# qiaozhijian/LPD-Net-Pytorch

Measured on AMD Instinct MI355X. Metric: global descriptors/sec (4096-pt clouds), higher is better.
Workload: dtype f32; 1 GPU; BASELINE configs[1]: LPD-Net (featnet=lpdnet, emb_dims=1024, no T-Nets) eval forward, N=4096, k=20, eval_batch_size=32 clouds/step/GPU; num_points=4096, batches_in_flight=2, parallelism=shard-by-cloud x1 (one process per GPU, no data-path collective)

## Files before the change

lpd-net-pytorch_amd/csrc/lpd_knn.hip:

```cpp
#include "lpd_common.h"
#include <math.h>
#include <type_traits>

namespace {

constexpr int KNN_WAVES = 4;
constexpr int KNN_THREADS = KNN_WAVES * 64;
constexpr int KNN_QPB = KNN_WAVES * 32;

template <int CP>
struct KnnCfg {
    static constexpr int CHUNK = (CP <= 32) ? 128 : (CP <= 64 ? 64 : 32);
    static constexpr int ROWS = 2 * CP;
    static constexpr int FLOATS = ROWS * CHUNK;
    static constexpr int PER_THREAD = FLOATS / KNN_THREADS;
};

__global__ void knn_sumsq_kernel(const float* __restrict__ x, float* __restrict__ xx, int C, int N)
{
    int n = blockIdx.x * blockDim.x + threadIdx.x;
    int b = blockIdx.y;
    if (n >= N) return;
    const float* p = x + (size_t)b * C * N + n;
    float total = 0.0f;
// ... 337 lines not shown
        knn_prep_bf16x8 e;
#pragma unroll
        for (int i = 0; i < 8; ++i) e[i] = (__bf16)0.0f;
        if (j == 0) {
            const float w = -0.5f * total;
            const __bf16 hi = (__bf16)w;
            e[0] = hi;
            e[1] = (__bf16)(w - (float)hi);
        }
        __bf16* f4 = xb + ((((size_t)b * nt + (pt >> 5)) * 5 + 4) * 64 + (pt & 31) + 32 * j) * 8;
        *reinterpret_cast<knn_prep_bf16x8*>(f4) = e;
    }
}

template <int CP>
__device__ __forceinline__ void knn3_ld_ops(const float* __restrict__ xpb, int N, int j, int h, float (&a)[CP])
{
    const float* row = xpb + ((size_t)min(j, N - 1) * 2 + h) * CP;
    if constexpr (CP % 4 == 0) {
#pragma unroll
        for (int g = 0; g < CP / 4; ++g) {
            const float4 v = *reinterpret_cast<const float4*>(row + 4 * g);
            a[4 * g + 0] = v.x; a[4 * g + 1] = v.y; a[4 * g + 2] = v.z; a[4 * g + 3] = v.w;
        }
    } else {
        const float2 v = *reinterpret_cast<const float2*>(row);
        a[0] = v.x; a[1] = v.y;
    }
}

__device__ __forceinline__ void knn3_ld_xx(const float* __restrict__ xxb, int N, int j0, int h, bool vec_ok, float4 (&x4)[4])
{
    if (vec_ok && j0 + 32 <= N) {
#pragma unroll
        for (int g = 0; g < 4; ++g) x4[g] = *reinterpret_cast<const float4*>(xxb + j0 + 8 * g + 4 * h);
        return;
    }
    const float nanv = __builtin_nanf("");
#pragma unroll
    for (int g = 0; g < 4; ++g) {
        const int r0 = j0 + 8 * g + 4 * h;
        x4[g].x = r0 + 0 < N ? xxb[r0 + 0] : nanv;
        x4[g].y = r0 + 1 < N ? xxb[r0 + 1] : nanv;
        x4[g].z = r0 + 2 < N ? xxb[r0 + 2] : nanv;
        x4[g].w = r0 + 3 < N ? xxb[r0 + 3] : nanv;
    }
}

template <int CP, bool ALWAYS = false>
__device__ __forceinline__ void knn3_tile(float (&a)[CP], float4 (&x4)[4], const float (&qreg)[CP], float xq,
                                          const float* __restrict__ xpb, const float* __restrict__ xxb, int N, int j_next,
                                          bool have_next, int col, int h, bool vec_ok, float (&pd)[16])
{
    if constexpr (ALWAYS) have_next = true;
    f32x16 acc = {0, 0, 0, 0, 0, 0, 0, 0, 0, 0, 0, 0, 0, 0, 0, 0};
    const float* row = xpb + ((size_t)min(j_next + col, N - 1) * 2 + h) * CP;
    if constexpr (CP % 4 == 0) {
#pragma unroll
        for (int g = 0; g < CP / 4; ++g) {
#pragma unroll
            for (int e = 0; e < 4; ++e)
                acc = __builtin_amdgcn_mfma_f32_32x32x2f32(a[4 * g + e], qreg[4 * g + e], acc, 0, 0, 0);
            if (have_next) {
                const float4 v = *reinterpret_cast<const float4*>(row + 4 * g);
                a[4 * g + 0] = v.x; a[4 * g + 1] = v.y; a[4 * g + 2] = v.z; a[4 * g + 3] = v.w;
            }
        }
    } else {
#pragma unroll
        for (int s = 0; s < CP; ++s) acc = __builtin_amdgcn_mfma_f32_32x32x2f32(a[s], qreg[s], acc, 0, 0, 0);
        if (have_next) {
            const float2 v = *reinterpret_cast<const float2*>(row);
            a[0] = v.x; a[1] = v.y;
        }
    }
#pragma unroll
    for (int r = 0; r < 16; ++r) {
        const float4 xv = x4[r >> 2];
        const float xxj = (r & 3) == 0 ? xv.x : (r & 3) == 1 ? xv.y : (r & 3) == 2 ? xv.z : xv.w;
        pd[r] = __fsub_rn(__fmaf_rn(2.0f, acc[r], -xxj), xq);
    }
    if constexpr (ALWAYS) {
#pragma unroll
        for (int g = 0; g < 4; ++g) x4[g] = *reinterpret_cast<const float4*>(xxb + j_next + 8 * g + 4 * h);
    } else if (have_next) knn3_ld_xx(xxb, N, j_next, h, vec_ok, x4);
}

template <int CP, int KMAX>
__global__ __launch_bounds__(KNN3_THREADS, ((KMAX > 32 || (KMAX == 32 && CP == 32)) ? 1 : 2))
void knn3_kernel(const float* __restrict__ xp, const float* __restrict__ xx, int32_t* __restrict__ idx, int N, int k,
                 int blocks_per_cloud, int dbg)
{
    extern __shared__ __attribute__((aligned(16))) float smem[];
    const int tid = threadIdx.x;
    const int lane = tid & 63;
    const int wave = tid >> 6;
    const int h = lane >> 5;
    const int col = lane & 31;
    const int vb = lpd_xcd_remap(blockIdx.x, gridDim.x);
    const int b = vb / blocks_per_cloud;
    const int qb = vb - b * blocks_per_cloud;
    const int q0 = qb * (KNN3_WAVES * 32) + wave * 32;
    const int q = q0 + col;
    const bool q_ok = q < N;
    const float* xpb = xp + (size_t)b * N * (2 * CP);
    const float* xxb = xx + (size_t)b * N;
    const bool vec_ok = (N & 3) == 0;
    float2* myq = reinterpret_cast<float2*>(smem + (size_t)wave * knn3_wave_floats<KMAX>()) + lane;

    float qreg[CP];
    knn3_ld_ops<CP>(xpb, N, q, h, qreg);
    const float xq = xxb[min(q, N - 1)];

    float lv[KMAX];
    int li[KMAX];
    auto reset_lists = [&]() {
#pragma unroll
        for (int s = 0; s < KMAX; ++s) {
            lv[s] = -INFINITY;
            li[s] = 0x7fffffff;
        }
    };
    reset_lists();

    const int ntiles = (N + 31) / 32;
    float a[CP];
    float4 x4[4];
    float pd[16];

    {
        const int t_own = q0 / 32;
        int t_lo = t_own - 1, t_hi = t_own + 2;
        while ((t_hi - t_lo) * 16 < KMAX) { --t_lo; ++t_hi; }
        if (t_lo < 0) { t_hi -= t_lo; t_lo = 0; }
        if (t_hi > ntiles) { t_lo -= t_hi - ntiles; t_hi = ntiles; }
        if (t_lo < 0) t_lo = 0;
        knn3_ld_ops<CP>(xpb, N, t_lo * 32 + col, h, a);
        knn3_ld_xx(xxb, N, t_lo * 32, h, vec_ok, x4);
        for (int t = t_lo; t < t_hi; ++t) {
            knn3_tile<CP>(a, x4, qreg, xq, xpb, xxb, N, (t + 1) * 32, t + 1 < t_hi, col, h, vec_ok, pd);
#pragma unroll
            for (int r = 0; r < 16; ++r) knn_insert_values<KMAX>(lv, pd[r] > lv[KMAX - 1] ? pd[r] : -INFINITY);
        }
    }
    float t0 = k <= KMAX ? lv[KMAX - 1] : -INFINITY;
    {
        const float other = __shfl_xor(t0, 32, 64);
        t0 = fmaxf(t0, other);
        if (!(t0 > -INFINITY)) t0 = -INFINITY;
    }
    reset_lists();

    int cnt = 0;
    int stat_adm = 0, stat_it = 0, stat_pass = 0;
    auto drain = [&]() {
        stat_adm += cnt;
        int nmax = cnt;
#pragma unroll
        for (int m = 32; m >= 1; m >>= 1) nmax = max(nmax, __shfl_xor(nmax, m, 64));
        nmax = __builtin_amdgcn_readfirstlane(nmax);
        for (int e = 0; e < nmax; ++e) {
            ++stat_it;
            const float2 ent = myq[(e < cnt ? e : 0) * 64];
            const float pv = (e < cnt && ent.x > lv[KMAX - 1]) ? ent.x : -INFINITY;
            knn_insert_inplace<KMAX>(lv, li, pv, __float_as_int(ent.y));
        }
        cnt = 0;
    };
    knn3_ld_ops<CP>(xpb, N, col, h, a);
    knn3_ld_xx(xxb, N, 0, h, vec_ok, x4);
    for (int t = 0; t < ntiles; ++t) {
        knn3_tile<CP>(a, x4, qreg, xq, xpb, xxb, N, (t + 1) * 32, (t + 1 < ntiles), col, h, vec_ok, pd);
        const float thr = fmaxf(t0, lv[KMAX - 1]);
        const bool list_full = lv[KMAX - 1] > -INFINITY;
        float mx = fmaxf(fmaxf(fmaxf(pd[0], pd[1]), fmaxf(pd[2], pd[3])), fmaxf(fmaxf(pd[4], pd[5]), fmaxf(pd[6], pd[7])));
        mx = fmaxf(mx, fmaxf(fmaxf(fmaxf(pd[8], pd[9]), fmaxf(pd[10], pd[11])), fmaxf(fmaxf(pd[12], pd[13]), fmaxf(pd[14], pd[15]))));
        if (!__any(list_full ? (mx > thr) : (mx >= thr))) continue;
        ++stat_pass;
#pragma unroll
        for (int r = 0; r < 16; ++r) {
            const bool admit = list_full ? (pd[r] > thr) : (pd[r] >= thr);
            if (admit) {
                const int row = (r & 3) + 8 * (r >> 2) + 4 * h;
                myq[cnt * 64] = make_float2(pd[r], __int_as_float(t * 32 + row));
                ++cnt;
            }
        }
        if (__any(cnt > KNN3_QCAP - 16)) drain();
    }
    drain();

    float* mv = smem + (size_t)wave * knn3_wave_floats<KMAX>();
    int* mi = reinterpret_cast<int*>(mv + 64 * KMAX);
#pragma unroll
    for (int s = 0; s < KMAX; ++s) {
        mv[lane * KMAX + s] = lv[s];
        mi[lane * KMAX + s] = li[s];
    }
    __syncthreads();
    if ((dbg & 64) && q_ok) {
        if (h == 0) { int32_t* o = idx + ((size_t)b * N + q) * k; o[0] = stat_adm; o[1] = stat_it; o[2] = stat_pass; o[3] = __float_as_int(t0); }
        else { int32_t* o = idx + ((size_t)b * N + q) * k; o[4] = stat_adm; }
    } else
    if (h == 0 && q_ok) {
        const float* av = mv + lane * KMAX;
        const int* ai = mi + lane * KMAX;
        const float* bv = mv + (lane + 32) * KMAX;
        const int* bi = mi + (lane + 32) * KMAX;
        int pa = 0, pb = 0;
        int32_t* out = idx + ((size_t)b * N + q) * k;
        for (int s = 0; s < k; ++s) {
            bool take_a;
            if (pa >= KMAX) take_a = false;
            else if (pb >= KMAX) take_a = true;
            else {
                const float va = av[pa], vb2 = bv[pb];
                take_a = (va > vb2) || (va == vb2 && ai[pa] < bi[pb]);
            }
            if (take_a) out[s] = ai[pa++];
            else out[s] = bi[pb++];
        }
    }
}

constexpr bool KNN7_DEFAULT = true;
constexpr int KNN7_QCAP = 24;
constexpr int KNN7_MAXT = 128;
constexpr int KNN7_WAVE_LDS = KNN7_MAXT * 32 * 2 + KNN7_QCAP * 64 * 8;
constexpr int KNN7_QCAP_XYZ = 20;
constexpr int KNN7_QCAP_BIG = 48;
constexpr int KNN7_WAVE_LDS_XYZ = KNN7_QCAP_XYZ * 64 * 8;
constexpr bool KNN7_ONFLY64 = false;
template <int CP, int KMAX, bool ONFLY> struct Knn7Cfg {
    static constexpr int QCAP = KMAX > 20 ? (CP == 2 ? 32 : KNN7_QCAP_BIG) : ((CP == 2) ? KNN7_QCAP_XYZ : KNN7_QCAP);
    static constexpr int QBYTES = QCAP * 64 * 8;
    static constexpr int TBYTES = ONFLY ? 0 : KNN7_MAXT * 32 * 2;
    static constexpr int MERGE = KMAX > 20 ? 0 : 64 * KMAX * 8;
    static constexpr int WAVE = (TBYTES + QBYTES) > MERGE ? (TBYTES + QBYTES) : MERGE;
    static constexpr int QOFF = TBYTES;
    static constexpr int WAVES_PER_SIMD = KMAX > 20 ? (CP == 2 ? 2 : 1) : (CP == 2 ? 4 : 2);
};

__device__ __forceinline__ bool knn_before(float av, int ai, float bv, int bi) { return av > bv || (av == bv && ai < bi); }

__device__ __forceinline__ void knn_merge_halves_bitonic(float (&v)[64], int (&id)[64])
{
#pragma unroll
    for (int s = 0; s < 32; ++s) {
        const int r = 63 - s;
        const float pv_r = __shfl_xor(v[r], 32, 64), pv_s = __shfl_xor(v[s], 32, 64);
        const int pi_r = __shfl_xor(id[r], 32, 64), pi_s = __shfl_xor(id[s], 32, 64);
        const bool ks = knn_before(v[s], id[s], pv_r, pi_r);
        const bool kr = knn_before(v[r], id[r], pv_s, pi_s);
        v[s] = ks ? v[s] : pv_r; id[s] = ks ? id[s] : pi_r;
        v[r] = kr ? v[r] : pv_s; id[r] = kr ? id[r] : pi_s;
    }
#pragma unroll
    for (int d = 32; d >= 1; d >>= 1)
#pragma unroll
        for (int s = 0; s < 64; ++s)
            if ((s & d) == 0) {
                const bool sw = knn_before(v[s + d], id[s + d], v[s], id[s]);
                const float tv = v[s]; const int ti = id[s];
                v[s] = sw ? v[s + d] : tv; id[s] = sw ? id[s + d] : ti;
                v[s + d] = sw ? tv : v[s + d]; id[s + d] = sw ? ti : id[s + d];
            }
}

constexpr int KNN7_XB = 80;
constexpr int KNN7_PRE_MAXT = 512;
typedef __bf16 knn_bf16x8 __attribute__((ext_vector_type(8)));

__global__ __launch_bounds__(256) void knn7_bf16_kernel(const float* __restrict__ xp, const float* __restrict__ xx, __bf16* __restrict__ xb,
                                                        int N, int nt)
{
    const int t = blockIdx.x * blockDim.x + threadIdx.x;
    if (t >= nt * 64) return;
    const int b = blockIdx.y;
    const int T = t >> 6, lane = t & 63, h = lane >> 5;
    const int pt = min(T * 32 + (lane & 31), N - 1);
    const float* src = xp + (((size_t)b * N + pt) * 2 + h) * 32;
    __bf16* dst = xb + (((size_t)b * nt + T) * 5 * 64 + lane) * 8;
#pragma unroll
    for (int g = 0; g < 4; ++g) {
        const float4 a = *reinterpret_cast<const float4*>(src + 8 * g), c = *reinterpret_cast<const float4*>(src + 8 * g + 4);
        knn_bf16x8 v;
        v[0] = (__bf16)a.x; v[1] = (__bf16)a.y; v[2] = (__bf16)a.z; v[3] = (__bf16)a.w;
        v[4] = (__bf16)c.x; v[5] = (__bf16)c.y; v[6] = (__bf16)c.z; v[7] = (__bf16)c.w;
        *reinterpret_cast<knn_bf16x8*>(dst + (size_t)g * 512) = v;
    }
    knn_bf16x8 e;
#pragma unroll
    for (int i = 0; i < 8; ++i) e[i] = (__bf16)0.0f;
    if (h == 0) {
        const float v = -0.5f * xx[(size_t)b * N + pt];
        const __bf16 hi = (__bf16)v;
        e[0] = hi;
        e[1] = (__bf16)(v - (float)hi);
    }
    *reinterpret_cast<knn_bf16x8*>(dst + (size_t)4 * 512) = e;
}

constexpr int KNN7_BQT = 2;
__global__ __launch_bounds__(256, 2) void knn7_bound_kernel(const __bf16* __restrict__ xb, const float* __restrict__ xx,
                                                            const float* __restrict__ txmax, uint16_t* __restrict__ ubq, int N, int nt, int C,
                                                            int tchunk)
{
    constexpr int QT = KNN7_BQT;
    const int tid = threadIdx.x, lane = tid & 63, wave = tid >> 6;
    const int h = lane >> 5, col = lane & 31;
    const int b = blockIdx.y;
    const int W0 = (blockIdx.x * 4 + wave) * QT;
    const __bf16* xbb = xb + ((size_t)b * nt * 5 * 64 + lane) * 8;
    const float* txb = txmax + (size_t)b * nt;
    float smax = 0.f;
    for (int t = lane; t < nt; t += 64) smax = fmaxf(smax, txb[t]);
#pragma unroll
    for (int m = 32; m >= 1; m >>= 1) smax = fmaxf(smax, __shfl_xor(smax, m, 64));
    const float E0 = 8.0f * (float)(C + 8) * 1.1920929e-7f * smax + 1e-30f;

    knn_bf16x8 qop[QT][4], ones;
    float xq[QT], kq[QT];
#pragma unroll
    for (int e = 0; e < 8; ++e) ones[e] = (__bf16)((h == 0 && e < 2) ? 1.0f : 0.0f);
#pragma unroll
    for (int i = 0; i < QT; ++i) {
        const int Wq = min(W0 + i, nt - 1);
#pragma unroll
        for (int s = 0; s < 4; ++s) qop[i][s] = *reinterpret_cast<const knn_bf16x8*>(xbb + ((size_t)Wq * 5 + s) * 512);
        xq[i] = xx[(size_t)b * N + min(Wq * 32 + col, N - 1)];
        kq[i] = (sqrtf(xq[i]) * 1.0001f + 1e-30f) * 7.9e-3f;
    }
    float pinf = INFINITY;
    asm volatile("" : "+v"(pinf));
    auto mx2 = [&](float a_, float b_) { return __builtin_amdgcn_fmed3f(a_, b_, pinf); };
    constexpr int RING = 4;
    knn_bf16x8 cop[RING][5];
    auto load_c = [&](int T, knn_bf16x8 (&c)[5]) {
        T = T < nt ? T : nt - 1;
#pragma unroll
        for (int s = 0; s < 5; ++s) c[s] = *reinterpret_cast<const knn_bf16x8*>(xbb + ((size_t)T * 5 + s) * 512);
    };
    __shared__ float stx[KNN7_PRE_MAXT];
    for (int t = tid; t < nt; t += 256) stx[t] = txb[t];
    __syncthreads();
    if (W0 >= nt) return;
    auto one_tile = [&](int T, const knn_bf16x8 (&c)[5]) {
        const float tx = stx[T];
        const float ncT = sqrtf(tx) * 1.0001f;
        const float cT = 2.0f * (tx * 7.62939453125e-6f + E0);
#pragma unroll
        for (int i = 0; i < QT; ++i) {
            f32x16 sa = {0, 0, 0, 0, 0, 0, 0, 0, 0, 0, 0, 0, 0, 0, 0, 0};
#pragma unroll
            for (int s = 0; s < 4; ++s) sa = __builtin_amdgcn_mfma_f32_32x32x16_bf16(c[s], qop[i][s], sa, 0, 0, 0);
            sa = __builtin_amdgcn_mfma_f32_32x32x16_bf16(c[4], ones, sa, 0, 0, 0);
            float m = mx2(mx2(mx2(sa[0], sa[1]), mx2(sa[2], sa[3])), mx2(mx2(sa[4], sa[5]), mx2(sa[6], sa[7])));
            m = mx2(m, mx2(mx2(mx2(sa[8], sa[9]), mx2(sa[10], sa[11])), mx2(mx2(sa[12], sa[13]), mx2(sa[14], sa[15]))));
            m = mx2(m, __shfl_xor(m, 32, 64));
            float ub = 2.0f * m - xq[i] + (2.0f * (kq[i] * ncT) + cT);
            ub += fabsf(ub) * 9.5367431640625e-7f;
            uint32_t bits = __float_as_uint(ub);
            bits = (ub <= 0.0f) ? (bits >> 16) : 0x7f80u;
            if (h == 0 && W0 + i < nt) ubq[(((size_t)b * nt + (W0 + i)) * nt + T) * 32 + col] = (uint16_t)bits;
        }
    };
    const int tbeg = blockIdx.z * tchunk, tend = min(nt, tbeg + tchunk);
#pragma unroll
    for (int d = 0; d < RING - 1; ++d) load_c(tbeg + d, cop[d]);
    for (int T0 = tbeg; T0 < tend; T0 += RING) {
#pragma unroll
        for (int d = 0; d < RING; ++d) {
            load_c(T0 + d + RING - 1, cop[(d + RING - 1) % RING]);
            if (T0 + d < tend) one_tile(T0 + d, cop[d]);
        }
    }
}

template <int CP>
__global__ __launch_bounds__(64) void knn7_tile_stats_kernel(const float* __restrict__ xp, const float* __restrict__ xx,
                                                            float* __restrict__ cenp, float* __restrict__ cnorm,
                                                            float* __restrict__ rad, float* __restrict__ txmax, int N, int nt)
{
    constexpr int CH = 2 * CP;
    __shared__ float cen[CH];
    const int t = blockIdx.x, b = blockIdx.y, tid = threadIdx.x;
    const int cnt = min(32, N - t * 32);
    const float* base = xp + ((size_t)b * N + (size_t)t * 32) * CH;
    for (int c = tid; c < CH; c += 64) {
        float sum = 0.f;
        for (int i = 0; i < cnt; ++i) sum += base[(size_t)i * CH + c];
        const float m = sum / (float)cnt;
        cen[c] = m;
        cenp[((size_t)b * nt + t) * CH + c] = m;
    }
    __syncthreads();
    float d2 = 0.f, nx = 0.f, cn = 0.f;
    if (tid < cnt) {
        for (int c = 0; c < CH; ++c) {
            const float d = base[(size_t)tid * CH + c] - cen[c];
            d2 = fmaf(d, d, d2);
        }
        nx = xx[(size_t)b * N + t * 32 + tid];
    }
    for (int c = tid; c < CH; c += 64) cn = fmaf(cen[c], cen[c], cn);
#pragma unroll
    for (int m = 32; m >= 1; m >>= 1) {
        d2 = fmaxf(d2, __shfl_xor(d2, m, 64));
        nx = fmaxf(nx, __shfl_xor(nx, m, 64));
        cn += __shfl_xor(cn, m, 64);
    }
    const bool bad = __any(tid < cnt && !(fabsf(xx[(size_t)b * N + t * 32 + tid]) <= 3.0e38f));
    if (tid == 0) {
        rad[(size_t)b * nt + t] = sqrtf(d2) * 1.0001f + 1e-30f;
        cnorm[(size_t)b * nt + t] = cn;
        txmax[(size_t)b * nt + t] = bad ? INFINITY : nx;
    }
}

template <int CP>
__global__ __launch_bounds__(128) void knn7_predict_kernel(const float* __restrict__ cenp, const float* __restrict__ rad,
                                                           int32_t* __restrict__ pred, int nt)
{
    constexpr int CH = 2 * CP;
    __shared__ float cw[CH];
    __shared__ int part[2];
    const int W = blockIdx.x, b = blockIdx.y, tid = threadIdx.x;
    const float* cb = cenp + (size_t)b * nt * CH;
    for (int c = tid; c < CH; c += 128) cw[c] = cb[(size_t)W * CH + c];
    __syncthreads();
    const float rw = rad[(size_t)b * nt + W];
    int n = 0;
    for (int T = tid; T < nt; T += 128) {
        const float* ct = cb + (size_t)T * CH;
        float d2 = 0.f;
        if constexpr (CH % 4 == 0) {
#pragma unroll 4
            for (int c = 0; c < CH; c += 4) {
                const float4 v = *reinterpret_cast<const float4*>(ct + c);
                const float d0 = v.x - cw[c], d1 = v.y - cw[c + 1], d2_ = v.z - cw[c + 2], d3 = v.w - cw[c + 3];
                d2 = fmaf(d0, d0, fmaf(d1, d1, fmaf(d2_, d2_, fmaf(d3, d3, d2))));
            }
        } else {
            for (int c = 0; c < CH; ++c) { const float d = ct[c] - cw[c]; d2 = fmaf(d, d, d2); }
        }
        const float gap = fmaxf(sqrtf(d2) - rw - rad[(size_t)b * nt + T], 0.0f);
        n += gap <= 0.5f * rw ? 1 : 0;
    }
#pragma unroll
    for (int m = 32; m >= 1; m >>= 1) n += __shfl_xor(n, m, 64);
    if ((tid & 63) == 0) part[tid >> 6] = n;
    __syncthreads();
    if (tid == 0) pred[(size_t)b * nt + W] = part[0] + part[1];
}

constexpr int KNN7_PRED_WPB = 16;
template <int CP>
__global__ __launch_bounds__(256) void knn7_predict_lds_kernel(const float* __restrict__ cenp, const float* __restrict__ rad,
                                                               int32_t* __restrict__ pred, int nt)
{
    constexpr int CH = 2 * CP, LD = CH + 1;
    extern __shared__ float pcen[];
    float* prad = pcen + (size_t)nt * LD;
    const int b = blockIdx.y, tid = threadIdx.x;
    const float* cb = cenp + (size_t)b * nt * CH;
    for (int i = tid; i < nt * CH; i += 256) pcen[(i / CH) * LD + (i % CH)] = cb[i];
    for (int i = tid; i < nt; i += 256) prad[i] = rad[(size_t)b * nt + i];
    __syncthreads();
    const int W = blockIdx.x * KNN7_PRED_WPB + (tid >> 4), l = tid & 15;
    const int Wc = min(W, nt - 1);
    const float* cw = pcen + (size_t)Wc * LD;
    const float rw = prad[Wc];
    int n = 0;
    for (int T = l; T < nt; T += 16) {
        const float* ct = pcen + (size_t)T * LD;
        float d2 = 0.f;
#pragma unroll 16
        for (int c = 0; c < CH; ++c) { const float d = ct[c] - cw[c]; d2 = fmaf(d, d, d2); }
        const float gap = fmaxf(sqrtf(d2) - rw - prad[T], 0.0f);
        n += gap <= 0.5f * rw ? 1 : 0;
    }
#pragma unroll
    for (int m = 8; m >= 1; m >>= 1) n += __shfl_xor(n, m, 64);
    if (l == 0 && W < nt) pred[(size_t)b * nt + W] = n;
}

__global__ __launch_bounds__(1024) void knn7_order_kernel(const int32_t* __restrict__ pred, int32_t* __restrict__ order, int nitems)
{
    __shared__ unsigned sk[1024];
    const int tid = threadIdx.x, xcd = blockIdx.y;
    const int q = nitems / 8, r = nitems % 8;
    const int base = xcd < r ? xcd * (q + 1) : r * (q + 1) + (xcd - r) * q;
    const int len = q + (xcd < r ? 1 : 0);
    const int c0 = blockIdx.x * 1024;
    if (c0 >= len) return;
    const int cl = min(1024, len - c0);
    unsigned v = ~0u;
    if (tid < cl) v = ((0xffffu - (unsigned)min(pred[base + c0 + tid], 0xfffe)) << 16) | (unsigned)tid;
    for (int k = 2; k <= 1024; k <<= 1) {
        for (int j = k >> 1; j > 0; j >>= 1) {
            unsigned o;
            if (j < 64) o = __shfl_xor(v, j, 64);
            else {
                sk[tid] = v;
                __syncthreads();
                o = sk[tid ^ j];
                __syncthreads();
            }
            const bool lower = (tid & j) == 0, up = (tid & k) == 0;
            const unsigned mn = v < o ? v : o, mx = v < o ? o : v;
            v = (lower == up) ? mn : mx;
        }
    }
    if (tid < cl) order[base + c0 + tid] = base + c0 + (int)(v & 0xffffu);
}

template <int KMAX>
__device__ __forceinline__ void knn7_insert(float (&v)[KMAX], int (&id)[KMAX], float x, float y, int j)
{
    unsigned long long cc, cp;
    int ti;
    asm volatile("v_cmp_ge_f32_e64 %0, %1, %2" : "=s"(cc) : "v"(v[KMAX - 1]), "v"(y));
#pragma unroll
    for (int s = KMAX - 1; s >= 1; --s) {
        asm volatile(
            "v_cmp_ge_f32_e64 %[cp], %[vp], %[y]\n\t"
            "v_med3_f32 %[vs], %[vp], %[vs], %[x]\n\t"
            "s_nop 0\n\t"
            "v_cndmask_b32_e64 %[ti], %[ip], %[j], %[cp]\n\t"
            "v_cndmask_b32_e64 %[is], %[ti], %[is], %[cc]"
            : [vs] "+v"(v[s]), [is] "+v"(id[s]), [cp] "=&s"(cp), [ti] "=&v"(ti)
            : [vp] "v"(v[s - 1]), [ip] "v"(id[s - 1]), [x] "v"(x), [y] "v"(y), [j] "v"(j), [cc] "s"(cc));
        cc = cp;
    }
    asm volatile(
        "v_cndmask_b32_e64 %[i0], %[j], %[i0], %[cc]\n\t"
        "v_max_f32 %[v0], %[v0], %[x]"
        : [v0] "+v"(v[0]), [i0] "+v"(id[0])
        : [x] "v"(x), [j] "v"(j), [cc] "s"(cc));
}

constexpr unsigned KNN_IMG_NINF = 0x00800000u;
constexpr unsigned KNN_IMG_EMPTY = 0u;
constexpr unsigned KNN_LOW_EMPTY = 0x80000000u;

__device__ __forceinline__ unsigned knn_img(float pd)
{
    const unsigned b = __float_as_uint(pd);
    return (int)b < 0 ? 0u - b : b ^ 0x80000000u;
}
__device__ __forceinline__ float knn_img_inv(unsigned im)
{
    im = im < KNN_IMG_NINF ? KNN_IMG_NINF : im;
    return __uint_as_float((im & 0x80000000u) ? im ^ 0x80000000u : 0u - im);
}

#define KNN_SUB_(n)  "v_sub_co_u32_e64 %[t], %[m" #n "], %[xl" #n "], %[yl" #n "]\n\t"
#define KNN_SBB_(n)  "v_subb_co_u32_e64 %[t], %[m" #n "], %[xh" #n "], %[yh" #n "], %[m" #n "]\n\t"
#define KNN_SELX_(n) "v_cndmask_b32_e64 %[nl" #n "], %[xl" #n "], %[yl" #n "], %[m" #n "]\n\t" \
                     "v_cndmask_b32_e64 %[nh" #n "], %[xh" #n "], %[yh" #n "], %[m" #n "]\n\t"
#define KNN_SELY_(n) "v_cndmask_b32_e64 %[yl" #n "], %[yl" #n "], %[xl" #n "], %[m" #n "]\n\t" \
                     "v_cndmask_b32_e64 %[yh" #n "], %[yh" #n "], %[xh" #n "], %[m" #n "]\n\t"
#define KNN_SELM_(n) "v_cndmask_b32_e64 %[xl" #n "], %[xl" #n "], %[yl" #n "], %[m" #n "]\n\t" \
                     "v_cndmask_b32_e64 %[xh" #n "], %[xh" #n "], %[yh" #n "], %[m" #n "]\n\t"
#define KNN_CXOUT_(n) [nl##n] "=&v"(nl##n), [nh##n] "=&v"(nh##n), [yl##n] "+v"(yl##n), [yh##n] "+v"(yh##n), [m##n] "=&s"(m##n)
#define KNN_CXIN_(n)  [xl##n] "v"(xl##n), [xh##n] "v"(xh##n)
#define KNN_MXOUT_(n) [xl##n] "+v"(xl##n), [xh##n] "+v"(xh##n), [m##n] "=&s"(m##n)
#define KNN_MXIN_(n)  [yl##n] "v"(yl##n), [yh##n] "v"(yh##n)
#define KNN_KEYREF_(n) unsigned &xh##n, unsigned &xl##n, unsigned &yh##n, unsigned &yl##n

__device__ __forceinline__ void knn_cx3(KNN_KEYREF_(0), KNN_KEYREF_(1), KNN_KEYREF_(2))
{
    unsigned long long m0, m1, m2;
    unsigned t, nl0, nh0, nl1, nh1, nl2, nh2;
    asm(KNN_SUB_(0) KNN_SUB_(1) KNN_SUB_(2) KNN_SBB_(0) KNN_SBB_(1) KNN_SBB_(2)
        KNN_SELX_(0) KNN_SELY_(0) KNN_SELX_(1) KNN_SELY_(1) KNN_SELX_(2) KNN_SELY_(2)
        : KNN_CXOUT_(0), KNN_CXOUT_(1), KNN_CXOUT_(2), [t] "=&v"(t)
        : KNN_CXIN_(0), KNN_CXIN_(1), KNN_CXIN_(2));
    xl0 = nl0; xh0 = nh0; xl1 = nl1; xh1 = nh1; xl2 = nl2; xh2 = nh2;
}
__device__ __forceinline__ void knn_cx2(KNN_KEYREF_(0), KNN_KEYREF_(1))
{
    unsigned long long m0, m1;
    unsigned t, nl0, nh0, nl1, nh1;
    asm(KNN_SUB_(0) KNN_SUB_(1) "s_nop 0\n\t" KNN_SBB_(0) KNN_SBB_(1) "s_nop 0\n\t"
        KNN_SELX_(0) KNN_SELY_(0) KNN_SELX_(1) KNN_SELY_(1)
        : KNN_CXOUT_(0), KNN_CXOUT_(1), [t] "=&v"(t)
        : KNN_CXIN_(0), KNN_CXIN_(1));
    xl0 = nl0; xh0 = nh0; xl1 = nl1; xh1 = nh1;
}
__device__ __forceinline__ void knn_cx1(KNN_KEYREF_(0))
{
    unsigned long long m0;
    unsigned t, nl0, nh0;
    asm(KNN_SUB_(0) "s_nop 1\n\t" KNN_SBB_(0) "s_nop 1\n\t" KNN_SELX_(0) KNN_SELY_(0)
        : KNN_CXOUT_(0), [t] "=&v"(t)
        : KNN_CXIN_(0));
    xl0 = nl0; xh0 = nh0;
}
__device__ __forceinline__ void knn_mx3(KNN_KEYREF_(0), KNN_KEYREF_(1), KNN_KEYREF_(2))
{
    unsigned long long m0, m1, m2;
    unsigned t;
    asm(KNN_SUB_(0) KNN_SUB_(1) KNN_SUB_(2) KNN_SBB_(0) KNN_SBB_(1) KNN_SBB_(2) KNN_SELM_(0) KNN_SELM_(1) KNN_SELM_(2)
        : KNN_MXOUT_(0), KNN_MXOUT_(1), KNN_MXOUT_(2), [t] "=&v"(t)
        : KNN_MXIN_(0), KNN_MXIN_(1), KNN_MXIN_(2));
}
__device__ __forceinline__ void knn_mx2(KNN_KEYREF_(0), KNN_KEYREF_(1))
{
    unsigned long long m0, m1;
    unsigned t;
    asm(KNN_SUB_(0) KNN_SUB_(1) "s_nop 0\n\t" KNN_SBB_(0) KNN_SBB_(1) "s_nop 0\n\t" KNN_SELM_(0) KNN_SELM_(1)
        : KNN_MXOUT_(0), KNN_MXOUT_(1), [t] "=&v"(t)
        : KNN_MXIN_(0), KNN_MXIN_(1));
}
__device__ __forceinline__ void knn_mx1(KNN_KEYREF_(0))
{
    unsigned long long m0;
    unsigned t;
    asm(KNN_SUB_(0) "s_nop 1\n\t" KNN_SBB_(0) "s_nop 1\n\t" KNN_SELM_(0)
        : KNN_MXOUT_(0), [t] "=&v"(t)
        : KNN_MXIN_(0));
}
#define KNN_K_(a, i) a##h[i], a##l[i]
#define KNN_CX3(a, i, b, j, c, k, d, l, e, m, f, n) knn_cx3(KNN_K_(a, i), KNN_K_(b, j), KNN_K_(c, k), KNN_K_(d, l), KNN_K_(e, m), KNN_K_(f, n))
#define KNN_CX2(a, i, b, j, c, k, d, l) knn_cx2(KNN_K_(a, i), KNN_K_(b, j), KNN_K_(c, k), KNN_K_(d, l))
#define KNN_CX1(a, i, b, j) knn_cx1(KNN_K_(a, i), KNN_K_(b, j))
#define KNN_MX3(a, i, b, j, c, k, d, l, e, m, f, n) knn_mx3(KNN_K_(a, i), KNN_K_(b, j), KNN_K_(c, k), KNN_K_(d, l), KNN_K_(e, m), KNN_K_(f, n))
#define KNN_MX2(a, i, b, j, c, k, d, l) knn_mx2(KNN_K_(a, i), KNN_K_(b, j), KNN_K_(c, k), KNN_K_(d, l))
#define KNN_MX1(a, i, b, j) knn_mx1(KNN_K_(a, i), KNN_K_(b, j))
#define KNN_PLACE(...) { constexpr int pl[20] = {__VA_ARGS__}; unsigned th[20], tl[20]; \
    _Pragma("unroll") for (int s = 0; s < 20; ++s) { th[s] = kh[pl[s]]; tl[s] = kl[pl[s]]; } \
    _Pragma("unroll") for (int s = 0; s < 20; ++s) { kh[s] = th[s]; kl[s] = tl[s]; } }

template <int NB> __device__ __forceinline__ void knn_merge_batch(unsigned (&kh)[20], unsigned (&kl)[20], unsigned (&bh)[NB], unsigned (&bl)[NB]);
template <> __device__ __forceinline__ void knn_merge_batch<8>(unsigned (&kh)[20], unsigned (&kl)[20], unsigned (&bh)[8], unsigned (&bl)[8])
{
    KNN_CX3(b, 0, b, 1,  b, 2, b, 3,  b, 4, b, 5);
    KNN_CX3(b, 6, b, 7,  b, 0, b, 2,  b, 1, b, 3);
    KNN_CX3(b, 4, b, 6,  b, 5, b, 7,  b, 1, b, 2);
    KNN_CX3(b, 5, b, 6,  b, 0, b, 4,  b, 3, b, 7);
    KNN_CX2(b, 1, b, 5,  b, 2, b, 6);
    KNN_CX2(b, 2, b, 4,  b, 3, b, 5);
    KNN_CX3(b, 1, b, 2,  b, 3, b, 4,  b, 5, b, 6);
    KNN_MX3(k, 12, b, 7,  k, 13, b, 6,  k, 14, b, 5);
    KNN_MX3(k, 15, b, 4,  k, 16, b, 3,  k, 17, b, 2);
    KNN_MX2(k, 18, b, 1,  k, 19, b, 0);
    KNN_CX3(k, 0, k, 16,  k, 1, k, 17,  k, 2, k, 18);
    KNN_CX3(k, 3, k, 19,  k, 16, k, 8,  k, 17, k, 9);
    KNN_CX3(k, 18, k, 10,  k, 19, k, 11,  k, 4, k, 12);
    KNN_CX3(k, 5, k, 13,  k, 6, k, 14,  k, 7, k, 15);
    KNN_CX3(k, 16, k, 4,  k, 17, k, 5,  k, 18, k, 6);
    KNN_CX3(k, 19, k, 7,  k, 8, k, 12,  k, 9, k, 13);
    KNN_CX3(k, 10, k, 14,  k, 11, k, 15,  k, 0, k, 2);
    KNN_CX3(k, 1, k, 3,  k, 16, k, 18,  k, 17, k, 19);
    KNN_CX3(k, 4, k, 6,  k, 5, k, 7,  k, 8, k, 10);
    KNN_CX3(k, 9, k, 11,  k, 12, k, 14,  k, 13, k, 15);
    KNN_CX3(k, 0, k, 1,  k, 2, k, 3,  k, 16, k, 17);
    KNN_CX3(k, 18, k, 19,  k, 4, k, 5,  k, 6, k, 7);
    KNN_CX3(k, 8, k, 9,  k, 10, k, 11,  k, 12, k, 13);
    KNN_CX1(k, 14, k, 15);
    KNN_PLACE(0, 1, 2, 3, 16, 17, 18, 19, 4, 5, 6, 7, 8, 9, 10, 11, 12, 13, 14, 15);
}
template <> __device__ __forceinline__ void knn_merge_batch<16>(unsigned (&kh)[20], unsigned (&kl)[20], unsigned (&bh)[16], unsigned (&bl)[16])
{
    KNN_CX3(b, 0, b, 1,  b, 2, b, 3,  b, 4, b, 5);
    KNN_CX3(b, 6, b, 7,  b, 8, b, 9,  b, 10, b, 11);
    KNN_CX3(b, 12, b, 13,  b, 14, b, 15,  b, 0, b, 2);
    KNN_CX3(b, 1, b, 3,  b, 4, b, 6,  b, 5, b, 7);
    KNN_CX3(b, 8, b, 10,  b, 9, b, 11,  b, 12, b, 14);
    KNN_CX3(b, 13, b, 15,  b, 1, b, 2,  b, 5, b, 6);
    KNN_CX3(b, 9, b, 10,  b, 13, b, 14,  b, 0, b, 4);
    KNN_CX3(b, 1, b, 5,  b, 2, b, 6,  b, 3, b, 7);
    KNN_CX3(b, 8, b, 12,  b, 9, b, 13,  b, 10, b, 14);
    KNN_CX3(b, 11, b, 15,  b, 2, b, 4,  b, 3, b, 5);
    KNN_CX3(b, 10, b, 12,  b, 11, b, 13,  b, 1, b, 2);
    KNN_CX3(b, 3, b, 4,  b, 5, b, 6,  b, 9, b, 10);
    KNN_CX3(b, 11, b, 12,  b, 13, b, 14,  b, 0, b, 8);
    KNN_CX3(b, 1, b, 9,  b, 2, b, 10,  b, 3, b, 11);
// ... 847 lines not shown
```

Baseline: 19860 descriptors/s.

## Software-pipeline kNN bound kernel with double-buffered MFMA accumulators and buffer loads

Restructures the kNN tile upper-bound kernel so that each step issues the MFMAs for the next tile while finishing the max-reduction and store for the previous tile, using two alternating accumulator sets. Per-tile constants are precomputed once into shared memory as float2. Global loads and stores go through raw buffer resources. The cross-half-wave shuffle is replaced by permlane32_swap, so each half-wave handles one query tile's store. Explicit sched_group_barrier hints interleave MFMA and VALU work. The aim is to hide MFMA latency and cut address and shuffle overhead, at the cost of more registers and a hand-written tail.

```diff
diff --git a/lpd-net-pytorch_amd/csrc/lpd_knn.hip b/lpd-net-pytorch_amd/csrc/lpd_knn.hip
--- a/lpd-net-pytorch_amd/csrc/lpd_knn.hip
+++ b/lpd-net-pytorch_amd/csrc/lpd_knn.hip
@@ -663,16 +663,85 @@
 }
 
 constexpr int KNN7_BQT = 2;
+constexpr int KNN7_BRING = 4;
+
+struct Knn7BoundCtx {
+    knn_bf16x8 qop[KNN7_BQT][4], ones;
+    float xqh, kqh, pinf;
+    const float2* sct;
+    __amdgpu_buffer_rsrc_t xres, ures;
+    unsigned xoff, uoff;
+    int nt;
+};
+
+__device__ __forceinline__ float knn7_mx2(const Knn7BoundCtx& k, float a, float b) { return __builtin_amdgcn_fmed3f(a, b, k.pinf); }
+
+__device__ __forceinline__ void knn7_bound_load(const Knn7BoundCtx& k, int T, knn_bf16x8 (&c)[5])
+{
+    T = T < k.nt ? T : k.nt - 1;
+#pragma unroll
+    for (int s = 0; s < 5; ++s) c[s] = __builtin_bit_cast(knn_bf16x8, __builtin_amdgcn_raw_buffer_load_b128(k.xres, k.xoff, (unsigned)(T * 5 + s) * 1024u, 0));
+}
+
+__device__ __forceinline__ void knn7_bound_mma(const Knn7BoundCtx& k, const knn_bf16x8 (&c)[5], f32x16 (&a)[KNN7_BQT])
+{
+#pragma unroll
+    for (int i = 0; i < KNN7_BQT; ++i) {
+        f32x16 sa = {0, 0, 0, 0, 0, 0, 0, 0, 0, 0, 0, 0, 0, 0, 0, 0};
+#pragma unroll
+        for (int s = 0; s < 4; ++s) sa = __builtin_amdgcn_mfma_f32_32x32x16_bf16(c[s], k.qop[i][s], sa, 0, 0, 0);
+        a[i] = __builtin_amdgcn_mfma_f32_32x32x16_bf16(c[4], k.ones, sa, 0, 0, 0);
+    }
+}
+
+__device__ __forceinline__ float knn7_bound_max16(const Knn7BoundCtx& k, const f32x16& sa)
+{
+    float p[8];
+#pragma unroll
+    for (int j = 0; j < 8; ++j) p[j] = knn7_mx2(k, sa[2 * j], sa[2 * j + 1]);
+    const float a = fmaxf(fmaxf(p[0], p[1]), p[2]), b = fmaxf(fmaxf(p[3], p[4]), p[5]);
+    return fmaxf(fmaxf(a, b), fmaxf(p[6], p[7]));
+}
+
+__device__ __forceinline__ void knn7_bound_finish(const Knn7BoundCtx& k, int T, const f32x16 (&a)[KNN7_BQT])
+{
+    const float m0 = knn7_bound_max16(k, a[0]), m1 = knn7_bound_max16(k, a[1]);
+    const auto r = __builtin_amdgcn_permlane32_swap(__float_as_uint(m0), __float_as_uint(m1), false, false);
+    const float m = knn7_mx2(k, __uint_as_float(r[0]), __uint_as_float(r[1]));
+    const float2 ct = k.sct[T];
+    float ub = fmaf(2.0f, m, -k.xqh) + fmaf(2.0f, k.kqh * ct.x, ct.y);
+    ub += fabsf(ub) * 9.5367431640625e-7f;
+    uint32_t bits = __float_as_uint(ub);
+    bits = (ub <= 0.0f) ? (bits >> 16) : 0x7f80u;
+    __builtin_amdgcn_raw_buffer_store_b16((unsigned short)bits, k.ures, k.uoff, (unsigned)T * 64u, 0);
+}
+
+template <bool LOAD>
+__device__ __forceinline__ void knn7_bound_step(const Knn7BoundCtx& k, int T, knn_bf16x8 (&cl)[5], const knn_bf16x8 (&c)[5],
+                                                f32x16 (&an)[KNN7_BQT], const f32x16 (&ap)[KNN7_BQT])
+{
+    if constexpr (LOAD) knn7_bound_load(k, T + KNN7_BRING, cl);
+    knn7_bound_mma(k, c, an);
+    knn7_bound_finish(k, T, ap);
+    __builtin_amdgcn_sched_group_barrier(0x100, 1, 0);
+#pragma unroll
+    for (int i = 0; i < 5 * KNN7_BQT; ++i) {
+        __builtin_amdgcn_sched_group_barrier(0x8, 1, 0);
+        __builtin_amdgcn_sched_group_barrier(0x2, 5, 0);
+    }
+}
+
 __global__ __launch_bounds__(256, 2) void knn7_bound_kernel(const __bf16* __restrict__ xb, const float* __restrict__ xx,
                                                             const float* __restrict__ txmax, uint16_t* __restrict__ ubq, int N, int nt, int C,
                                                             int tchunk)
 {
-    constexpr int QT = KNN7_BQT;
-    const int tid = threadIdx.x, lane = tid & 63, wave = tid >> 6;
+    constexpr int QT = KNN7_BQT, RING = KNN7_BRING;
+    static_assert(QT == 2 && RING % 2 == 0, "two query tiles (one per half-wave at the store); accumulator sets alternate with the ring");
+    const int tid = threadIdx.x, lane = tid & 63;
+    const int wave = __builtin_amdgcn_readfirstlane(tid >> 6);
     const int h = lane >> 5, col = lane & 31;
     const int b = blockIdx.y;
     const int W0 = (blockIdx.x * 4 + wave) * QT;
-    const __bf16* xbb = xb + ((size_t)b * nt * 5 * 64 + lane) * 8;
     const float* txb = txmax + (size_t)b * nt;
     float smax = 0.f;
     for (int t = lane; t < nt; t += 64) smax = fmaxf(smax, txb[t]);
@@ -680,62 +749,55 @@
     for (int m = 32; m >= 1; m >>= 1) smax = fmaxf(smax, __shfl_xor(smax, m, 64));
     const float E0 = 8.0f * (float)(C + 8) * 1.1920929e-7f * smax + 1e-30f;
 
-    knn_bf16x8 qop[QT][4], ones;
-    float xq[QT], kq[QT];
-#pragma unroll
-    for (int e = 0; e < 8; ++e) ones[e] = (__bf16)((h == 0 && e < 2) ? 1.0f : 0.0f);
+    __shared__ float2 sct[KNN7_PRE_MAXT];
+    for (int t = tid; t < nt; t += 256) {
+        const float tx = txb[t];
+        sct[t] = make_float2(sqrtf(tx) * 1.0001f, 2.0f * (tx * 7.62939453125e-6f + E0));
+    }
+    __syncthreads();
+    if (W0 >= nt) return;
+
+    Knn7BoundCtx k;
+    k.nt = nt;
+    k.sct = sct;
+    k.xres = __builtin_amdgcn_make_buffer_rsrc(reinterpret_cast<unsigned char*>(const_cast<__bf16*>(xb)) + (size_t)b * nt * 5 * 1024, 0,
+                                               (unsigned)nt * 5 * 1024, 0x00020000);
+    k.xoff = lane * 16;
+#pragma unroll
+    for (int e = 0; e < 8; ++e) k.ones[e] = (__bf16)((h == 0 && e < 2) ? 1.0f : 0.0f);
 #pragma unroll
     for (int i = 0; i < QT; ++i) {
         const int Wq = min(W0 + i, nt - 1);
 #pragma unroll
-        for (int s = 0; s < 4; ++s) qop[i][s] = *reinterpret_cast<const knn_bf16x8*>(xbb + ((size_t)Wq * 5 + s) * 512);
-        xq[i] = xx[(size_t)b * N + min(Wq * 32 + col, N - 1)];
-        kq[i] = (sqrtf(xq[i]) * 1.0001f + 1e-30f) * 7.9e-3f;
-    }
-    float pinf = INFINITY;
-    asm volatile("" : "+v"(pinf));
-    auto mx2 = [&](float a_, float b_) { return __builtin_amdgcn_fmed3f(a_, b_, pinf); };
-    constexpr int RING = 4;
+        for (int s = 0; s < 4; ++s) k.qop[i][s] = __builtin_bit_cast(knn_bf16x8, __builtin_amdgcn_raw_buffer_load_b128(k.xres, k.xoff, (unsigned)(Wq * 5 + s) * 1024u, 0));
+    }
+    const int Wh = min(W0 + h, nt - 1);
+    k.xqh = xx[(size_t)b * N + min(Wh * 32 + col, N - 1)];
+    k.kqh = (sqrtf(k.xqh) * 1.0001f + 1e-30f) * 7.9e-3f;
+    k.ures = __builtin_amdgcn_make_buffer_rsrc(reinterpret_cast<unsigned char*>(ubq) + (size_t)b * nt * nt * 64, 0, (unsigned)nt * nt * 64, 0x00020000);
+    k.uoff = ((unsigned)Wh * nt * 32 + col) * 2;
+    k.pinf = INFINITY;
+    asm volatile("" : "+v"(k.pinf));
+
+    const int tbeg = blockIdx.z * tchunk, tend = min(nt, tbeg + tchunk);
+    if (tbeg >= tend) return;
     knn_bf16x8 cop[RING][5];
-    auto load_c = [&](int T, knn_bf16x8 (&c)[5]) {
-        T = T < nt ? T : nt - 1;
-#pragma unroll
-        for (int s = 0; s < 5; ++s) c[s] = *reinterpret_cast<const knn_bf16x8*>(xbb + ((size_t)T * 5 + s) * 512);
-    };
-    __shared__ float stx[KNN7_PRE_MAXT];
-    for (int t = tid; t < nt; t += 256) stx[t] = txb[t];
-    __syncthreads();
-    if (W0 >= nt) return;
-    auto one_tile = [&](int T, const knn_bf16x8 (&c)[5]) {
-        const float tx = stx[T];
-        const float ncT = sqrtf(tx) * 1.0001f;
-        const float cT = 2.0f * (tx * 7.62939453125e-6f + E0);
-#pragma unroll
-        for (int i = 0; i < QT; ++i) {
-            f32x16 sa = {0, 0, 0, 0, 0, 0, 0, 0, 0, 0, 0, 0, 0, 0, 0, 0};
-#pragma unroll
-            for (int s = 0; s < 4; ++s) sa = __builtin_amdgcn_mfma_f32_32x32x16_bf16(c[s], qop[i][s], sa, 0, 0, 0);
-            sa = __builtin_amdgcn_mfma_f32_32x32x16_bf16(c[4], ones, sa, 0, 0, 0);
-            float m = mx2(mx2(mx2(sa[0], sa[1]), mx2(sa[2], sa[3])), mx2(mx2(sa[4], sa[5]), mx2(sa[6], sa[7])));
-            m = mx2(m, mx2(mx2(mx2(sa[8], sa[9]), mx2(sa[10], sa[11])), mx2(mx2(sa[12], sa[13]), mx2(sa[14], sa[15]))));
-            m = mx2(m, __shfl_xor(m, 32, 64));
-            float ub = 2.0f * m - xq[i] + (2.0f * (kq[i] * ncT) + cT);
-            ub += fabsf(ub) * 9.5367431640625e-7f;
-            uint32_t bits = __float_as_uint(ub);
-            bits = (ub <= 0.0f) ? (bits >> 16) : 0x7f80u;
-            if (h == 0 && W0 + i < nt) ubq[(((size_t)b * nt + (W0 + i)) * nt + T) * 32 + col] = (uint16_t)bits;
-        }
-    };
-    const int tbeg = blockIdx.z * tchunk, tend = min(nt, tbeg + tchunk);
-#pragma unroll
-    for (int d = 0; d < RING - 1; ++d) load_c(tbeg + d, cop[d]);
-    for (int T0 = tbeg; T0 < tend; T0 += RING) {
-#pragma unroll
-        for (int d = 0; d < RING; ++d) {
-            load_c(T0 + d + RING - 1, cop[(d + RING - 1) % RING]);
-            if (T0 + d < tend) one_tile(T0 + d, cop[d]);
-        }
-    }
+    f32x16 acc[2][QT];
+#pragma unroll
+    for (int d = 0; d < RING; ++d) knn7_bound_load(k, tbeg + d, cop[d]);
+    knn7_bound_mma(k, cop[0], acc[0]);
+    int T0 = tbeg;
+    for (; T0 + RING < tend; T0 += RING) {
+#pragma unroll
+        for (int d = 0; d < RING; ++d) knn7_bound_step<true>(k, T0 + d, cop[d], cop[(d + 1) % RING], acc[(d + 1) & 1], acc[d & 1]);
+    }
+    static_assert(RING == 4, "the tail below is written out for four sets");
+    const int left = tend - T0;
+    if (left > 1) knn7_bound_step<false>(k, T0, cop[0], cop[1], acc[1], acc[0]);
+    if (left > 2) knn7_bound_step<false>(k, T0 + 1, cop[1], cop[2], acc[0], acc[1]);
+    if (left > 3) knn7_bound_step<false>(k, T0 + 2, cop[2], cop[3], acc[1], acc[0]);
+    if (left & 1) knn7_bound_finish(k, tend - 1, acc[0]);
+    else knn7_bound_finish(k, tend - 1, acc[1]);
 }
 
 template <int CP>
```

After: 20090 descriptors/s (median of 6 runs). +1.2%, better.
